# kongzhecn/OMG

Hardware: NVIDIA H100
Metric: 1024^2 images/sec @30 steps, 2 concepts (higher is better)
Workload: dtype f16

## Files before the change

### omg_b200/csrc/gemm_tc.cu

```cuda
#include <cuda_fp16.h>
#include <stdlib.h>
#include <string.h>

#include <algorithm>
#include <type_traits>

#include "../../include/omg_b200.h"
#include "elem.cuh"
#include "host_common.h"
#include "ptx.cuh"
#include "wgmma.cuh"

namespace omg {

constexpr int BM = 128;
constexpr int BK = 64;
constexpr int GEMM_THREADS = 384;

struct SegDev {
    int a_map, dx, dy, a_c0, k_blocks, b_k0, b_map;
};

struct alignas(64) GemmParams {
    CUtensorMap a_maps[OMG_MAX_A];
    CUtensorMap b_maps[2];
    SegDev segs[OMG_MAX_SEGS];
    int n_segs;
    int units;
    int n_units;
    int tw, th, tiles_w, tiles_h;
    int img_w, img_h, img_b;
    int N, N_out;
    void* out;
    long long out_sw, out_sh, out_sb;
    const void* bias;
    const void* rowvec;
    int rowvec_ld;
    const void* residual;
    int residual_ld;
    int act_silu;
    float* stats_out;
    int stats_unit_planes;
    const float* stats_in;
    int stats_parts;
    long long stats_rows;
    float ln_inv_dim, ln_eps;
    const float* col_c1;
    const float* col_c2;
    int n_col_groups;
    long long col_group_end[8];
    int w_group_rows;
    const float* residual_f32;
    long long residual_f32_ld;
    float* out_f32;
    long long out_f32_ld;
    float4* col_stats;
    int cs_rb0, cs_rb_total;
};

template <int UN, bool CS>
struct GemmCfg {
    static constexpr int ACC = UN;
    static constexpr int A_BYTES = BM * BK * 2;
    static constexpr int B_BYTES = UN * BK * 2;
    static constexpr int STAGE_BYTES = A_BYTES + B_BYTES;
    static constexpr int VEC_BYTES = 2 * 2 * UN * 4;
    static constexpr int CS_BYTES = CS ? 2 * 8 * (UN / 2) * 16 : 0;
    static constexpr int BARS_BYTES = 256;
    static constexpr int BUDGET = 227 * 1024 - 1024  - VEC_BYTES - CS_BYTES - BARS_BYTES;
    static constexpr int STAGES_RAW = BUDGET / STAGE_BYTES;
    static constexpr int STAGES = STAGES_RAW > 8 ? 8 : STAGES_RAW;
    static constexpr int SMEM_BYTES = 1024 + STAGES * STAGE_BYTES + VEC_BYTES + CS_BYTES + BARS_BYTES;
    static_assert(STAGES >= 2, "shared memory budget");
    static_assert((2 * STAGES + 2) * 8 <= BARS_BYTES, "barrier space");
};

__device__ __forceinline__ float gelu_exact(float x) { return 0.5f * x * (1.0f + erff(x * 0.70710678118654752f)); }

template <typename T, int WN>
__device__ __forceinline__ void wgmma_ss(float* d, uint64_t da, uint64_t db) {
    if constexpr (std::is_same_v<T, __nv_bfloat16>) {
        if constexpr (WN == 64) wgmma_ss_n64_bf16(*reinterpret_cast<float(*)[32]>(d), da, db, 1u);
        else if constexpr (WN == 128) wgmma_ss_n128_bf16(*reinterpret_cast<float(*)[64]>(d), da, db, 1u);
        else wgmma_ss_n160_bf16(*reinterpret_cast<float(*)[80]>(d), da, db, 1u);
    } else {
        if constexpr (WN == 64) wgmma_ss_n64(*reinterpret_cast<float(*)[32]>(d), da, db, 1u);
        else if constexpr (WN == 128) wgmma_ss_n128(*reinterpret_cast<float(*)[64]>(d), da, db, 1u);
        else wgmma_ss_n160(*reinterpret_cast<float(*)[80]>(d), da, db, 1u);
    }
}

template <int STAGES>
__device__ __forceinline__ void ring_advance(int& stage, uint32_t& phase, int n) {
    stage += n;
    const int wraps = stage / STAGES;
    stage -= wraps * STAGES;
    phase ^= (uint32_t)wraps & 1u;
}

template <typename T, int UN, int EPI, int FEAT>
__global__ void __launch_bounds__(GEMM_THREADS, 1) gemm_tc_kernel(const __grid_constant__ GemmParams p) {
    using T2 = pair_t<T>;
    constexpr bool kStats = FEAT >= 1, kExtra = FEAT >= 2;
    static_assert(EPI != OMG_EPI_GEGLU || UN == 160, "GEGLU runs on 160-wide units");
    using Cfg = GemmCfg<UN, kStats>;
    constexpr int STAGES = Cfg::STAGES;
    constexpr int NJ = UN / 8;
    extern __shared__ __align__(1024) uint8_t smem_raw[];
    uint8_t* smem = reinterpret_cast<uint8_t*>((reinterpret_cast<uintptr_t>(smem_raw) + 1023) & ~uintptr_t(1023));
    float* s_vec = reinterpret_cast<float*>(smem + STAGES * Cfg::STAGE_BYTES);
    float4* s_cs_all = reinterpret_cast<float4*>(s_vec + 2 * 2 * UN);
    uint64_t* full_bar = reinterpret_cast<uint64_t*>(reinterpret_cast<uint8_t*>(s_cs_all) + Cfg::CS_BYTES);
    uint64_t* empty_bar = full_bar + STAGES;
    uint64_t* turn_bar = empty_bar + STAGES;

    const int warp = threadIdx.x >> 5;
    const int lane = threadIdx.x & 31;
    const int tiles_per_img = p.tiles_w * p.tiles_h;

    if (warp == 8 && lane == 0) {
        for (int i = 0; i < OMG_MAX_A; ++i) tma_prefetch_desc(&p.a_maps[i]);
        tma_prefetch_desc(&p.b_maps[0]);
        tma_prefetch_desc(&p.b_maps[1]);
        for (int i = 0; i < STAGES; ++i) {
            mbar_init(&full_bar[i], 1);
            mbar_init(&empty_bar[i], 1);
        }
        mbar_init(&turn_bar[0], 1);
        mbar_init(&turn_bar[1], 1);
        fence_barrier_init();
    }
    __syncthreads();
    griddep_launch_dependents();
    griddep_wait();

    if (warp >= 8) {
        asm volatile("setmaxnreg.dec.sync.aligned.u32 40;");
        if (warp == 8 && lane == 0) {
            int stage = 0;
            uint32_t phase = 0;
            for (int u = blockIdx.x; u < p.units; u += gridDim.x) {
                const int m_tile = u / p.n_units, nu = u % p.n_units;
                const int b = m_tile / tiles_per_img;
                const int rem = m_tile % tiles_per_img;
                const int h0 = (rem / p.tiles_w) * p.th, w0 = (rem % p.tiles_w) * p.tw;
                int n0 = nu * UN;
                if (p.w_group_rows > 0) {
                    const long long tile_pix0 = ((long long)b * p.img_h + h0) * p.img_w + w0;
                    for (int g2 = 0; g2 + 1 < p.n_col_groups; ++g2)
                        if (tile_pix0 >= p.col_group_end[g2]) n0 += p.w_group_rows;
                }
                for (int s = 0; s < p.n_segs; ++s) {
                    const SegDev sg = p.segs[s];
                    for (int kb = 0; kb < sg.k_blocks; ++kb) {
                        mbar_wait_nocall(&empty_bar[stage], phase ^ 1);
                        uint8_t* a_dst = smem + stage * Cfg::STAGE_BYTES;
                        uint8_t* b_dst = a_dst + Cfg::A_BYTES;
                        mbar_arrive_expect_tx(&full_bar[stage], Cfg::STAGE_BYTES);
                        tma_load_4d(a_dst, &p.a_maps[sg.a_map], &full_bar[stage], sg.a_c0 + kb * BK, w0 + sg.dx, h0 + sg.dy, b);
                        tma_load_2d(b_dst, &p.b_maps[sg.b_map], &full_bar[stage], sg.b_k0 + kb * BK, n0);
                        if (++stage == STAGES) {
                            stage = 0;
                            phase ^= 1;
                        }
                    }
                }
            }
        }
        return;
    }

    asm volatile("setmaxnreg.inc.sync.aligned.u32 232;");
    const int wg = warp >> 2;
    const int wi = warp & 3;
    const int g = lane >> 2, c = lane & 3;
    const int wtid = threadIdx.x & 127;
    float* s_bias = s_vec + wg * (2 * UN);
    float* s_c1 = s_bias + UN;
    float4* s_cs = s_cs_all + wg * (8 * (UN / 2));
    int unit_kb = 0;
    for (int s = 0; s < p.n_segs; ++s) unit_kb += p.segs[s].k_blocks;
    int stage = 0;
    uint32_t phase = 0;
    if (wg == 1) ring_advance<STAGES>(stage, phase, unit_kb);
    uint32_t turn_phase = wg == 0 ? 1u : 0u;
    float acc[Cfg::ACC];

    for (int u = blockIdx.x + wg * gridDim.x; u < p.units; u += 2 * gridDim.x) {
        const int m_tile = u / p.n_units, nu = u % p.n_units;
        const int n0 = nu * UN;
        const int b = m_tile / tiles_per_img;
        const int rem = m_tile % tiles_per_img;
        const int h0 = (rem / p.tiles_w) * p.th, w0 = (rem % p.tiles_w) * p.tw;
        const bool ln = p.stats_in != nullptr;

        named_bar_sync(1 + wg, 128);
        {
            size_t cg = 0;
            if (ln && p.n_col_groups > 1) {
                const long long tile_pix0 = ((long long)b * p.img_h + h0) * p.img_w + w0;
                for (int g2 = 0; g2 + 1 < p.n_col_groups; ++g2)
                    if (tile_pix0 >= p.col_group_end[g2]) cg = g2 + 1;
                cg *= (size_t)p.N;
            }
            for (int j = wtid; j < UN; j += 128) {
                float v = 0.f, c1 = 0.f;
                const int n = n0 + j;
                if (n < p.N) {
                    if (ln) {
                        v = p.col_c2[cg + n];
                        c1 = p.col_c1[cg + n];
                    } else {
                        if (p.bias) v += to_f32(static_cast<const T*>(p.bias)[n]);
                        if (p.rowvec && b < p.img_b) v += to_f32(static_cast<const T*>(p.rowvec)[(size_t)b * p.rowvec_ld + n]);
                    }
                }
                s_bias[j] = v;
                s_c1[j] = c1;
            }
        }
        named_bar_sync(1 + wg, 128);

#pragma unroll
        for (int i = 0; i < Cfg::ACC; ++i) acc[i] = 0.f;
        mbar_wait_nocall(&turn_bar[wg], turn_phase);
        turn_phase ^= 1;
        int prev_stage = -1;
        for (int s = 0; s < p.n_segs; ++s) {
            const int kbs = p.segs[s].k_blocks;
            for (int kb = 0; kb < kbs; ++kb) {
                mbar_wait_nocall(&full_bar[stage], phase);
                const uint32_t a_addr = smem_u32(smem + stage * Cfg::STAGE_BYTES);
                const uint32_t b_addr = a_addr + Cfg::A_BYTES;
                wgmma_fence();
#pragma unroll
                for (int k = 0; k < BK / 16; ++k) {
                    const uint64_t b_desc = gmma_desc_sw128(b_addr + k * 32, 1024, 16);
#pragma unroll
                    for (int i = 0; i < 2; ++i)
                        wgmma_ss<T, UN>(acc + i * (UN / 2), gmma_desc_sw128(a_addr + i * (64 * BK * 2) + k * 32, 1024, 16), b_desc);
                }
                wgmma_commit();
                wgmma_wait<1>();
                if (prev_stage >= 0 && wtid == 0) mbar_arrive(&empty_bar[prev_stage]);
                prev_stage = stage;
                if (++stage == STAGES) {
                    stage = 0;
                    phase ^= 1;
                }
            }
        }
        if (wtid == 0) mbar_arrive(&turn_bar[wg ^ 1]);
        wgmma_wait<0>();
        reg_fence(acc);
        if (wtid == 0) mbar_arrive(&empty_bar[prev_stage]);
        ring_advance<STAGES>(stage, phase, unit_kb);

#pragma unroll
        for (int blk = 0; blk < 2; ++blk) {
            float* a = acc + blk * (UN / 2);
            float row_sum[2] = {0.f, 0.f}, row_sq[2] = {0.f, 0.f};
            bool valid[2];
            size_t pix[2];
            T* orow[2];
            float ln_a[2] = {1.f, 1.f}, ln_k[2] = {0.f, 0.f};
#pragma unroll
            for (int h = 0; h < 2; ++h) {
                const int et = blk * 64 + wi * 16 + g + 8 * h;
                const int ph = h0 + et / p.tw, pw = w0 + et % p.tw;
                valid[h] = (ph < p.img_h) && (pw < p.img_w) && (b < p.img_b);
                pix[h] = ((size_t)b * p.img_h + ph) * p.img_w + pw;
                orow[h] = static_cast<T*>(p.out) + (long long)b * p.out_sb + (long long)ph * p.out_sh + (long long)pw * p.out_sw;
                if (ln && valid[h]) {
                    float sa = 0.f, sq = 0.f;
                    for (int t = 0; t < p.stats_parts; ++t) {
                        const float2 st = __ldg(reinterpret_cast<const float2*>(p.stats_in) + (size_t)t * p.stats_rows + pix[h]);
                        sa += st.x;
                        sq += st.y;
                    }
                    const float mu = sa * p.ln_inv_dim;
                    ln_a[h] = rsqrtf(fmaxf(sq * p.ln_inv_dim - mu * mu, 0.f) + p.ln_eps);
                    ln_k[h] = -ln_a[h] * mu;
                }
            }
            float4* cs_slot = s_cs + (size_t)(blk * 4 + wi) * (UN / 2);
#pragma unroll
            for (int J = 0; J < NJ; ++J) {
                const int col = 8 * J + 2 * c;
                const int n = n0 + col;
                float x[2][2];
// ... 8 lines not shown
#pragma unroll
                    for (int h = 0; h < 2; ++h) {
                        const float o = x[h][0] * gelu_exact(x[h][1]);
                        const float o_nb = __shfl_down_sync(0xffffffffu, o, 1);
                        if ((c & 1) == 0 && valid[h] && n < p.N)
                            *reinterpret_cast<T2*>(orow[h] + (n >> 1)) = from_f32x2<T>(o, o_nb);
                    }
                } else {
                    if constexpr (kExtra) {
#pragma unroll
                        for (int h = 0; h < 2; ++h)
#pragma unroll
                            for (int e = 0; e < 2; ++e) {
                                float v = x[h][e];
                                if (p.act_silu == 1) {
                                    v = v / (1.0f + __expf(-v));
                                } else if (p.act_silu == 2) {
                                    v = v / (1.0f + __expf(-1.702f * v));
                                } else if (p.act_silu == 3) {
                                    v = gelu_exact(v);
                                } else if (p.act_silu == 4) {
                                    const float u = 0.7978845608028654f * fmaf(0.044715f * v * v, v, v);
                                    v = 0.5f * v * (2.0f - __fdividef(2.0f, 1.0f + __expf(2.0f * u)));
                                } else if (p.act_silu == 5) {
                                    v = fmaxf(v, 0.f);
                                }
                                x[h][e] = v;
                            }
                    }
                    float4 cs = make_float4(0.f, 0.f, 0.f, 0.f);
#pragma unroll
                    for (int h = 0; h < 2; ++h) {
                        const bool ok = valid[h] && n < p.N;
                        if (ok && p.residual != nullptr) {
                            const float2 r = to_f32x2(*reinterpret_cast<const T2*>(static_cast<const T*>(p.residual) + pix[h] * (size_t)p.residual_ld + n));
                            x[h][0] += r.x;
                            x[h][1] += r.y;
                        }
                        if constexpr (kExtra) {
                            if (ok && p.residual_f32 != nullptr) {
                                const float2 r = *reinterpret_cast<const float2*>(p.residual_f32 + pix[h] * (size_t)p.residual_f32_ld + n);
                                x[h][0] += r.x;
                                x[h][1] += r.y;
                            }
                            if (ok && p.out_f32 != nullptr)
                                *reinterpret_cast<float2*>(p.out_f32 + pix[h] * (size_t)p.out_f32_ld + n) = make_float2(x[h][0], x[h][1]);
                        }
                        if (ok) {
                            row_sum[h] += x[h][0] + x[h][1];
                            row_sq[h] = fmaf(x[h][0], x[h][0], fmaf(x[h][1], x[h][1], row_sq[h]));
                        }
                        const T2 o = from_f32x2<T>(x[h][0], x[h][1]);
                        if (ok) *reinterpret_cast<T2*>(orow[h] + n) = o;
                        if constexpr (kStats) {
                            const float2 f = valid[h] ? to_f32x2(o) : make_float2(0.f, 0.f);
                            cs.x += f.x;
                            cs.y = fmaf(f.x, f.x, cs.y);
                            cs.z += f.y;
                            cs.w = fmaf(f.y, f.y, cs.w);
                        }
                    }
                    if constexpr (kStats) {
                        if (p.col_stats != nullptr) {
#pragma unroll
                            for (int off = 4; off < 32; off <<= 1) {
                                cs.x += __shfl_xor_sync(0xffffffffu, cs.x, off);
                                cs.y += __shfl_xor_sync(0xffffffffu, cs.y, off);
                                cs.z += __shfl_xor_sync(0xffffffffu, cs.z, off);
                                cs.w += __shfl_xor_sync(0xffffffffu, cs.w, off);
                            }
                            if (g == 0) cs_slot[4 * J + c] = cs;
                        }
                    }
                }
            }
            if constexpr (EPI != OMG_EPI_GEGLU) {
                if (p.stats_out != nullptr) {
                    float2* so = reinterpret_cast<float2*>(p.stats_out);
                    const int kp = p.stats_unit_planes, plane0 = nu * kp;
#pragma unroll
                    for (int h = 0; h < 2; ++h) {
                        float s = row_sum[h], q = row_sq[h];
                        s += __shfl_xor_sync(0xffffffffu, s, 1);
                        q += __shfl_xor_sync(0xffffffffu, q, 1);
                        s += __shfl_xor_sync(0xffffffffu, s, 2);
                        q += __shfl_xor_sync(0xffffffffu, q, 2);
                        if (c == 0 && valid[h]) {
                            so[(size_t)plane0 * p.stats_rows + pix[h]] = make_float2(s, q);
                            for (int t = 1; t < kp; ++t) so[(size_t)(plane0 + t) * p.stats_rows + pix[h]] = make_float2(0.f, 0.f);
                        }
                    }
                }
            }
            if constexpr (EPI != OMG_EPI_GEGLU && kStats) {
                if (p.col_stats != nullptr) {
                    named_bar_sync(3 + wg * 2 + (wi >> 1), 64);
                    const int q = blk * 2 + (wi >> 1);
                    const float4* s0 = s_cs + (size_t)(blk * 4 + (wi & 2)) * (UN / 2);
                    const float4* s1 = s0 + UN / 2;
                    if (b < p.img_b) {
                        const size_t rb = (size_t)b * p.cs_rb_total + p.cs_rb0 + (size_t)rem * 4 + q;
                        for (int cp = (wi & 1) * 32 + lane; cp < UN / 2; cp += 64) {
                            const int col = n0 + 2 * cp;
                            if (col < p.N) {
                                const float4 u4 = s0[cp], w4 = s1[cp];
                                p.col_stats[(rb * p.N + col) >> 1] = make_float4(u4.x + w4.x, u4.y + w4.y, u4.z + w4.z, u4.w + w4.w);
                            }
                        }
                    }
                }
            }
        }
    }
}

static int view_to_tmap(CUtensorMap* m, const omg_view4& v, CUtensorMapDataType dt, uint32_t box_c, uint32_t box_w,
                        uint32_t box_h, CUtensorMapSwizzle sw) {
    const uint64_t dims[4] = {(uint64_t)v.C, (uint64_t)v.W, (uint64_t)v.H, (uint64_t)v.B};
    const uint64_t strides[4] = {1, (uint64_t)v.sw, (uint64_t)v.sh, (uint64_t)v.sb};
    const uint32_t box[4] = {box_c, box_w, box_h, 1};
    return make_tmap(m, dt, v.ptr, 4, dims, strides, box, sw);
}

template <typename T, int UN, int EPI, int FEAT>
static int launch_gemm_f(const GemmParams& p, cudaStream_t stream) {
    using Cfg = GemmCfg<UN, (FEAT >= 1)>;
    static bool configured = false;
    static int num_sms = 0;
    if (!configured) {
        OMG_CUDA(cudaFuncSetAttribute(gemm_tc_kernel<T, UN, EPI, FEAT>, cudaFuncAttributeMaxDynamicSharedMemorySize,
                                      Cfg::SMEM_BYTES));
        int dev = 0;
        OMG_CUDA(cudaGetDevice(&dev));
        OMG_CUDA(cudaDeviceGetAttribute(&num_sms, cudaDevAttrMultiProcessorCount, dev));
        configured = true;
    }
    const int grid = std::min(p.units, num_sms);
    OMG_CUDA(launch_pdl(gemm_tc_kernel<T, UN, EPI, FEAT>, dim3(grid), dim3(GEMM_THREADS), Cfg::SMEM_BYTES, stream, p));
    return check_launch("gemm_tc_kernel");
}

template <int UN, int EPI>
static int launch_gemm(const GemmParams& p, cudaStream_t stream) {
    if constexpr (EPI == OMG_EPI_GEGLU) {
        return launch_gemm_f<__half, UN, EPI, 0>(p, stream);
    } else {
        if (p.act_silu != 0 || p.residual_f32 != nullptr || p.out_f32 != nullptr) return launch_gemm_f<__half, UN, EPI, 2>(p, stream);
        if (p.col_stats != nullptr) return launch_gemm_f<__half, UN, EPI, 1>(p, stream);
        return launch_gemm_f<__half, UN, EPI, 0>(p, stream);
    }
}

constexpr int PLAN_SMS = 132;
constexpr double TILE_OVERHEAD = 48.0;
static double tile_time(long tiles, double cols) {
    return (double)((tiles + PLAN_SMS - 1) / PLAN_SMS) * (cols + TILE_OVERHEAD);
}

constexpr long K_PLAN_LONG = 1000;
static int pick_block_n(int N, int epilogue, long m_tiles, long k_plan) {
    if (epilogue == OMG_EPI_GEGLU) return 256;
    const int cands[5] = {256, 160, 128, 64, 160};
    int best = 256;
    double best_t = 1e30;
    for (int i = 0; i < 5; ++i) {
        const bool pair = i == 4;
        if (pair && (k_plan < 16 || m_tiles < 2)) continue;
        const long nt = (N + cands[i] - 1) / cands[i];
        const long mt = pair ? (m_tiles + 1) / 2 : m_tiles;
        const double t = tile_time(nt * mt, pair ? 2.0 * cands[i] : cands[i]);
        if (t < best_t - 1e-9) {
            best_t = t;
            best = cands[i];
        }
    }
    return best;
}

}

using namespace omg;

// ... 43 lines not shown
    const bool silu = d->epilogue == OMG_EPI_SILU;
    const int act = silu ? 1 : (d->epilogue == OMG_EPI_QUICK_GELU ? 2 : (d->epilogue == OMG_EPI_GELU ? 3 : (d->epilogue == OMG_EPI_GELU_TANH ? 4 :
                    (d->epilogue == OMG_EPI_RELU ? 5 : 0))));
    OMG_CHECK(d->epilogue == OMG_EPI_NONE || geglu || act, "omg_gemm: unknown epilogue %d", d->epilogue);
    const int N_out = geglu ? d->N / 2 : d->N;
    OMG_CHECK(d->d.C == N_out, "omg_gemm: output view has %d channels, expected %d", d->d.C, N_out);
    OMG_CHECK(!geglu || (d->N % 64 == 0 && !d->residual && !d->rowvec),
              "omg_gemm: GEGLU needs N %% 64 == 0 and no residual/rowvec");
    OMG_CHECK(!d->residual || (N_out % 32 == 0 && d->residual_ld % 8 == 0),
              "omg_gemm: residual needs N %% 32 == 0 and ld %% 8 == 0");

    GemmParams p;
    memset(&p, 0, sizeof(p));
    const int W = d->d.W, H = d->d.H, B = d->d.B;
    OMG_CHECK(W >= 1 && H >= 1 && B >= 1, "omg_gemm: empty output grid");
    int tw = 128;
    while (tw / 2 >= W && tw > 1) tw /= 2;
    const int th = 128 / tw;
    p.tw = tw;
    p.th = th;
    p.tiles_w = (W + tw - 1) / tw;
    p.tiles_h = (H + th - 1) / th;
    p.img_w = W;
    p.img_h = H;
    p.img_b = B;
    const int m_tiles = p.tiles_w * p.tiles_h * B;
    p.N = d->N;
    p.N_out = N_out;
    const long k_blocks_hint = (long)(d->Ktot + (d->w2 ? d->K2tot : 0)) / 64;
    int bn = d->block_n ? d->block_n
                        : pick_block_n(d->N, d->epilogue, m_tiles, d->row_stats_out ? K_PLAN_LONG : k_blocks_hint);
    OMG_CHECK(bn == 64 || bn == 128 || bn == 160 || bn == 256 || bn == 320, "omg_gemm: block_n=%d unsupported", bn);
    OMG_CHECK(bn != 320 || (!geglu && d->N % 320 == 0), "omg_gemm: block_n=320 needs N %% 320 == 0 and no GEGLU");
    OMG_CHECK(d->cta_pair == 0 || d->cta_pair == 1 || d->cta_pair == 3, "omg_gemm: cta_pair=%d unsupported (0, 1 or 3)",
              d->cta_pair);
    if (geglu) bn = 256;
    const int unit_n = geglu ? 160 : (bn > 160 ? bn / 2 : bn);
    const int tile_units = geglu ? 1 : bn / unit_n;
    p.n_units = geglu ? (d->N + 159) / 160 : (d->N + bn - 1) / bn * tile_units;
    p.units = m_tiles * p.n_units;
    p.stats_unit_planes = (bn == 320 ? 4 : 2) / tile_units;
    p.bias = d->bias;
    p.rowvec = d->rowvec;
    p.rowvec_ld = d->rowvec_ld;
    p.residual = d->residual;
    p.residual_ld = d->residual_ld;
    p.act_silu = act;
    p.stats_out = static_cast<float*>(d->row_stats_out);
    p.stats_in = static_cast<const float*>(d->row_stats_in);
    p.stats_parts = d->row_stats_parts;
    p.stats_rows = d->row_stats_stride > 0 ? d->row_stats_stride : (long long)W * H * B;
    p.ln_inv_dim = d->ln_dim > 0 ? 1.0f / (float)d->ln_dim : 0.f;
    p.ln_eps = d->ln_eps;
    p.col_c1 = static_cast<const float*>(d->col_c1);
    p.col_c2 = static_cast<const float*>(d->col_c2);
    p.n_col_groups = d->n_col_groups > 0 ? d->n_col_groups : 1;
    p.w_group_rows = d->w_group_planes > 0 ? d->N : 0;
    OMG_CHECK(d->w_group_planes == 0 || d->w_group_planes == p.n_col_groups, "omg_gemm: w_group_planes must equal n_col_groups");
    OMG_CHECK(p.n_col_groups <= 8, "omg_gemm: at most 8 column-vector row groups");
    OMG_CHECK(d->w_group_planes == 0 || !d->w2, "omg_gemm: weight planes do not extend to the second weight matrix (w2)");
    const long long img_pix = (long long)W * H;
    for (int i = 0; i < 8; ++i) {
        p.col_group_end[i] = d->col_group_end[i];
        if (i + 1 >= p.n_col_groups) continue;
        if (H > 1)
            OMG_CHECK(d->col_group_end[i] % img_pix == 0,
                      "omg_gemm: row-group boundary %lld is inside an image of the %d x %d output grid (boundaries are "
                      "multiples of %lld pixels)", (long long)d->col_group_end[i], W, H, img_pix);
        else
            OMG_CHECK(d->col_group_end[i] % 128 == 0, "omg_gemm: row-group boundary %lld is not a multiple of the 128-row tile",
                      (long long)d->col_group_end[i]);
    }
    OMG_CHECK(!p.stats_in || (p.col_c1 && p.col_c2 && d->ln_dim > 0 && d->row_stats_parts >= 1 && !d->rowvec),
              "omg_gemm: folded LayerNorm needs col_c1, col_c2, ln_dim, row_stats_parts and no rowvec");
    OMG_CHECK(!p.stats_out || !geglu, "omg_gemm: row statistics cannot be emitted by the GEGLU epilogue");
    p.residual_f32 = static_cast<const float*>(d->residual_f32);
    p.residual_f32_ld = d->residual_f32_ld;
    p.out_f32 = static_cast<float*>(d->out_f32);
    p.out_f32_ld = d->out_f32_ld;
    OMG_CHECK((!p.residual_f32 && !p.out_f32) || (!geglu && d->N % 32 == 0 && !(d->residual && d->residual_f32)),
              "omg_gemm: fp32 residual / output twins need a non-GEGLU epilogue, N %% 32 == 0, and replace the fp16 residual");
    OMG_CHECK((!p.residual_f32 || d->residual_f32_ld % 4 == 0) && (!p.out_f32 || d->out_f32_ld % 4 == 0),
              "omg_gemm: fp32 twin row strides must be multiples of 4");
    OMG_CHECK((!p.residual_f32 && !p.out_f32) || (d->d.sw == d->d.C && d->d.sh == (int64_t)d->d.sw * W && d->d.sb == d->d.sh * H),
              "omg_gemm: fp32 twins need a contiguous output view (rows are indexed by pixel)");
    p.col_stats = static_cast<float4*>(d->col_stats_out);
    p.cs_rb0 = d->col_stats_rb0;
    p.cs_rb_total = d->col_stats_rb_total;
    OMG_CHECK(!p.col_stats || (!geglu && d->N % 32 == 0 && d->col_stats_rb0 >= 0 &&
                               d->col_stats_rb0 + p.tiles_w * p.tiles_h * 4 <= d->col_stats_rb_total),
              "omg_gemm: column statistics need a non-GEGLU epilogue, N %% 32 == 0 and rb0 + blocks <= rb_total");
    OMG_CHECK((!p.stats_out && !p.stats_in) || (d->d.sw == d->d.C && d->d.sh == (int64_t)d->d.sw * W && d->d.sb == d->d.sh * H),
              "omg_gemm: row statistics need a contiguous output view");

    for (int i = 0; i < d->n_a; ++i) {
        OMG_CHECK(d->a[i].ptr != nullptr, "omg_gemm: A view %d is null", i);
        if (view_to_tmap(&p.a_maps[i], d->a[i], tdt, BK, tw, th, CU_TENSOR_MAP_SWIZZLE_128B)) return 1;
    }
    for (int i = d->n_a; i < OMG_MAX_A; ++i) p.a_maps[i] = p.a_maps[0];
    {
        const uint64_t planes = d->w_group_planes > 0 ? (uint64_t)d->w_group_planes : 1;
        const uint64_t dims[2] = {(uint64_t)d->Ktot, (uint64_t)d->N * planes};
        const uint64_t strides[2] = {1, (uint64_t)d->Ktot};
        const uint32_t box[2] = {BK, (uint32_t)unit_n};
        if (make_tmap(&p.b_maps[0], tdt, d->w, 2, dims, strides, box, CU_TENSOR_MAP_SWIZZLE_128B)) return 1;
        p.b_maps[1] = p.b_maps[0];
    }
    if (d->w2 != nullptr) {
        OMG_CHECK(d->K2tot >= 8 && d->K2tot % 8 == 0, "omg_gemm: K2tot=%d must be a positive multiple of 8", d->K2tot);
        const uint64_t dims[2] = {(uint64_t)d->K2tot, (uint64_t)d->N};
        const uint64_t strides[2] = {1, (uint64_t)d->K2tot};
        const uint32_t box[2] = {BK, (uint32_t)unit_n};
        if (make_tmap(&p.b_maps[1], tdt, d->w2, 2, dims, strides, box, CU_TENSOR_MAP_SWIZZLE_128B)) return 1;
    }
    OMG_CHECK(d->d.sw % 2 == 0 && d->d.sh % 2 == 0 && d->d.sb % 2 == 0 && (reinterpret_cast<uintptr_t>(d->d.ptr) & 3) == 0,
              "omg_gemm: output view must be 4 B aligned per pixel");
    p.out = const_cast<void*>(d->d.ptr);
    p.out_sw = d->d.sw;
    p.out_sh = d->d.sh;
    p.out_sb = d->d.sb;

    p.n_segs = d->n_segs;
    for (int s = 0; s < d->n_segs; ++s) {
        const omg_seg& sg = d->segs[s];
        OMG_CHECK(sg.a_idx >= 0 && sg.a_idx < d->n_a, "omg_gemm: segment %d references A view %d", s, sg.a_idx);
        OMG_CHECK(sg.k_len > 0 && sg.a_c0 >= 0 && sg.b_k0 >= 0 && sg.a_c0 + sg.k_len <= d->a[sg.a_idx].C,
                  "omg_gemm: segment %d has a bad K range", s);
        OMG_CHECK(sg.b_idx == 0 || (sg.b_idx == 1 && d->w2 != nullptr), "omg_gemm: segment %d has a bad b_idx", s);
        const int ktot_s = sg.b_idx ? d->K2tot : d->Ktot;
        OMG_CHECK(sg.b_k0 + sg.k_len <= ktot_s, "omg_gemm: segment %d exceeds weight K (%d + %d > %d)", s, sg.b_k0,
                  sg.k_len, ktot_s);
        OMG_CHECK(sg.k_len % BK == 0 || sg.a_c0 + sg.k_len == d->a[sg.a_idx].C,
                  "omg_gemm: segment %d: K tail must end at the A view's last channel", s);
        p.segs[s] = SegDev{sg.a_idx, sg.dx, sg.dy, sg.a_c0, (sg.k_len + BK - 1) / BK, sg.b_k0, sg.b_idx};
    }

    if (bf16) {
        switch (unit_n) {
            case 64: return launch_gemm_f<__nv_bfloat16, 64, OMG_EPI_NONE, 0>(p, stream);
            case 128: return launch_gemm_f<__nv_bfloat16, 128, OMG_EPI_NONE, 0>(p, stream);
            default: return launch_gemm_f<__nv_bfloat16, 160, OMG_EPI_NONE, 0>(p, stream);
        }
    }
    if (geglu) return launch_gemm<160, OMG_EPI_GEGLU>(p, stream);
    switch (unit_n) {
        case 64: return launch_gemm<64, OMG_EPI_NONE>(p, stream);
        case 128: return launch_gemm<128, OMG_EPI_NONE>(p, stream);
        default: return launch_gemm<160, OMG_EPI_NONE>(p, stream);
    }
}

extern "C" int omg_gemm(const omg_gemm_desc* d, void* stream_) {
    const int rc = gemm_impl(d, stream_);
    if (rc == 0 && ::omg::plan_recording()) {
        const omg_gemm_desc c = *d;
        ::omg::plan_note([c](void* s) { return gemm_impl(&c, s); });
    }
    return rc;
}
```

### omg_b200/csrc/ptx.cuh

```cuda
#pragma once
#include <cuda.h>
#include <cuda_fp16.h>
#include <cuda_runtime.h>
#include <stdint.h>
#include <stdio.h>

namespace omg {

__device__ __forceinline__ uint32_t smem_u32(const void* p) {
    return static_cast<uint32_t>(__cvta_generic_to_shared(p));
}

__device__ __forceinline__ uint32_t lane_id() { return threadIdx.x & 31; }

__device__ __forceinline__ bool elect_one() {
    uint32_t pred;
    asm volatile(
        "{\n\t.reg .pred p;\n\t"
        "elect.sync _|p, 0xffffffff;\n\t"
        "selp.u32 %0, 1, 0, p;\n\t}\n"
        : "=r"(pred));
    return pred != 0;
}

__device__ __forceinline__ void griddep_launch_dependents() { asm volatile("griddepcontrol.launch_dependents;" ::: "memory"); }
__device__ __forceinline__ void griddep_wait() { asm volatile("griddepcontrol.wait;" ::: "memory"); }

__device__ __forceinline__ void mbar_init(uint64_t* bar, uint32_t count) {
    asm volatile("mbarrier.init.shared::cta.b64 [%0], %1;" ::"r"(smem_u32(bar)), "r"(count));
}
__device__ __forceinline__ void fence_barrier_init() {
    asm volatile("fence.mbarrier_init.release.cluster;" ::: "memory");
}
__device__ __forceinline__ void fence_proxy_async_smem() {
    asm volatile("fence.proxy.async.shared::cta;" ::: "memory");
}
__device__ __forceinline__ void mbar_arrive_expect_tx(uint64_t* bar, uint32_t bytes) {
    asm volatile("mbarrier.arrive.expect_tx.shared::cta.b64 _, [%0], %1;" ::"r"(smem_u32(bar)), "r"(bytes)
                 : "memory");
}
__device__ __forceinline__ void mbar_arrive(uint64_t* bar) {
    asm volatile("mbarrier.arrive.shared::cta.b64 _, [%0];" ::"r"(smem_u32(bar)) : "memory");
}
__device__ __forceinline__ bool mbar_try_wait(uint64_t* bar, uint32_t parity) {
    uint32_t ok;
    asm volatile(
        "{\n\t.reg .pred p;\n\t"
        "mbarrier.try_wait.parity.shared::cta.b64 p, [%1], %2;\n\t"
        "selp.u32 %0, 1, 0, p;\n\t}\n"
        : "=r"(ok)
        : "r"(smem_u32(bar)), "r"(parity)
        : "memory");
    return ok != 0;
}
#ifndef OMG_MBAR_TIMEOUT_CYCLES
#define OMG_MBAR_TIMEOUT_CYCLES (4000000000LL)
#endif
#ifndef OMG_MBAR_SUSPEND_NS
#define OMG_MBAR_SUSPEND_NS 20000
#endif
__device__ __forceinline__ bool mbar_try_wait_long(uint64_t* bar, uint32_t parity) {
    uint32_t ok;
    asm volatile(
        "{\n\t.reg .pred p;\n\t"
        "mbarrier.try_wait.parity.shared::cta.b64 p, [%1], %2, %3;\n\t"
        "selp.u32 %0, 1, 0, p;\n\t}\n"
        : "=r"(ok)
        : "r"(smem_u32(bar)), "r"(parity), "r"((uint32_t)OMG_MBAR_SUSPEND_NS)
        : "memory");
    return ok != 0;
}
__device__ __forceinline__ void mbar_wait(uint64_t* bar, uint32_t parity) {
    if (mbar_try_wait(bar, parity)) return;
    const long long t0 = clock64();
    uint32_t spins = 0;
    while (!mbar_try_wait_long(bar, parity)) {
        if ((++spins & 0x3FF) == 0 && clock64() - t0 > OMG_MBAR_TIMEOUT_CYCLES) {
            printf("omg: mbarrier timeout block=(%d,%d,%d) thread=%d bar=%u parity=%u\n", (int)blockIdx.x,
                   (int)blockIdx.y, (int)blockIdx.z, (int)threadIdx.x, smem_u32(bar), parity);
            __trap();
        }
    }
}

__device__ __forceinline__ void mbar_wait_nocall(uint64_t* bar, uint32_t parity) {
    if (mbar_try_wait(bar, parity)) return;
    const long long t0 = clock64();
    uint32_t spins = 0;
    while (!mbar_try_wait_long(bar, parity))
        if ((++spins & 0x3FF) == 0 && clock64() - t0 > OMG_MBAR_TIMEOUT_CYCLES) __trap();
}

__device__ __forceinline__ float fast_exp2(float x) {
    float y;
    asm("ex2.approx.ftz.f32 %0, %1;" : "=f"(y) : "f"(x));
    return y;
}

__device__ __forceinline__ void tma_prefetch_desc(const CUtensorMap* m) {
    asm volatile("prefetch.tensormap [%0];" ::"l"(reinterpret_cast<uint64_t>(m)) : "memory");
}
__device__ __forceinline__ void tma_load_2d(void* smem_dst, const CUtensorMap* m, uint64_t* bar, int c0, int c1) {
    asm volatile(
        "cp.async.bulk.tensor.2d.shared::cluster.global.mbarrier::complete_tx::bytes [%0], [%1, {%3, %4}], [%2];"
        ::"r"(smem_u32(smem_dst)), "l"(reinterpret_cast<uint64_t>(m)), "r"(smem_u32(bar)), "r"(c0), "r"(c1)
        : "memory");
}
__device__ __forceinline__ void tma_load_3d(void* smem_dst, const CUtensorMap* m, uint64_t* bar, int c0, int c1,
                                            int c2) {
    asm volatile(
        "cp.async.bulk.tensor.3d.shared::cluster.global.mbarrier::complete_tx::bytes [%0], [%1, {%3, %4, %5}], [%2];"
        ::"r"(smem_u32(smem_dst)), "l"(reinterpret_cast<uint64_t>(m)), "r"(smem_u32(bar)), "r"(c0), "r"(c1), "r"(c2)
        : "memory");
}
__device__ __forceinline__ void tma_load_4d(void* smem_dst, const CUtensorMap* m, uint64_t* bar, int c0, int c1,
                                            int c2, int c3) {
    asm volatile(
        "cp.async.bulk.tensor.4d.shared::cluster.global.mbarrier::complete_tx::bytes [%0], [%1, {%3, %4, %5, %6}], "
        "[%2];"
        ::"r"(smem_u32(smem_dst)), "l"(reinterpret_cast<uint64_t>(m)), "r"(smem_u32(bar)), "r"(c0), "r"(c1), "r"(c2),
        "r"(c3)
        : "memory");
}
__device__ __forceinline__ void tma_store_3d(const CUtensorMap* m, const void* smem_src, int c0, int c1, int c2) {
    asm volatile("cp.async.bulk.tensor.3d.global.shared::cta.bulk_group [%0, {%2, %3, %4}], [%1];" ::"l"(
                     reinterpret_cast<uint64_t>(m)),
                 "r"(smem_u32(smem_src)), "r"(c0), "r"(c1), "r"(c2)
                 : "memory");
}
__device__ __forceinline__ void tma_store_4d(const CUtensorMap* m, const void* smem_src, int c0, int c1, int c2,
                                             int c3) {
    asm volatile("cp.async.bulk.tensor.4d.global.shared::cta.bulk_group [%0, {%2, %3, %4, %5}], [%1];" ::"l"(
                     reinterpret_cast<uint64_t>(m)),
                 "r"(smem_u32(smem_src)), "r"(c0), "r"(c1), "r"(c2), "r"(c3)
                 : "memory");
}
__device__ __forceinline__ void tma_store_commit() { asm volatile("cp.async.bulk.commit_group;" ::: "memory"); }
template <int N>
__device__ __forceinline__ void tma_store_wait_read() {
    asm volatile("cp.async.bulk.wait_group.read %0;" ::"n"(N) : "memory");
// ... 8 lines not shown
    d |= static_cast<uint64_t>((smem_addr & 0x3FFFF) >> 4);
    d |= static_cast<uint64_t>((lbo_bytes >> 4) & 0x3FFF) << 16;
    d |= static_cast<uint64_t>((sbo_bytes >> 4) & 0x3FFF) << 32;
    d |= static_cast<uint64_t>(1) << 62;
    return d;
}
__device__ __forceinline__ uint64_t gmma_desc_sw32(uint32_t smem_addr) {
    uint64_t d = 0;
    d |= static_cast<uint64_t>((smem_addr & 0x3FFFF) >> 4);
    d |= static_cast<uint64_t>(256 >> 4) << 16;
    d |= static_cast<uint64_t>(256 >> 4) << 32;
    d |= static_cast<uint64_t>(3) << 62;
    return d;
}
__device__ __forceinline__ void wgmma_fence() { asm volatile("wgmma.fence.sync.aligned;" ::: "memory"); }
__device__ __forceinline__ void wgmma_commit() { asm volatile("wgmma.commit_group.sync.aligned;" ::: "memory"); }
template <int N>
__device__ __forceinline__ void wgmma_wait() {
    asm volatile("wgmma.wait_group.sync.aligned %0;" ::"n"(N) : "memory");
}
template <int N>
__device__ __forceinline__ void reg_fence(float (&r)[N]) {
#pragma unroll
    for (int i = 0; i < N; ++i) asm volatile("" : "+f"(r[i])::"memory");
}
__device__ __forceinline__ void named_bar_sync(int id, int count) {
    asm volatile("bar.sync %0, %1;" ::"r"(id), "r"(count) : "memory");
}

__device__ __forceinline__ void st_shared_v4(uint32_t addr, uint32_t a, uint32_t b, uint32_t c, uint32_t d) {
    asm volatile("st.shared.v4.b32 [%0], {%1, %2, %3, %4};" ::"r"(addr), "r"(a), "r"(b), "r"(c), "r"(d) : "memory");
}

__device__ __forceinline__ uint32_t pack_half2(float a, float b) {
    __half2 h = __floats2half2_rn(a, b);
    return *reinterpret_cast<uint32_t*>(&h);
}

}
```

Before: 0.1969.

## Pair CTAs in 2-CTA clusters and multicast the weight tiles via TMA

Adds an optional 2-CTA cluster mode for the persistent wgmma GEMM. Two CTAs take adjacent M tiles with the same N unit, and each loads half of the shared B (weight) tile, multicasting it to both CTAs. Empty barriers now need an arrival from both CTAs, and the producer drains the ring before exiting. The mode is on by default when N > 1280 and the row-group boundaries are even. It halves weight traffic from L2 per CTA, at the cost of cross-CTA coupling, cluster scheduling limits and extra remote barrier arrivals.

New measurement: 0.1997, median of 6. +1.4%, better.

```diff
diff --git a/omg_b200/csrc/gemm_tc.cu b/omg_b200/csrc/gemm_tc.cu
--- a/omg_b200/csrc/gemm_tc.cu
+++ b/omg_b200/csrc/gemm_tc.cu
@@ -26,6 +26,7 @@
     CUtensorMap b_maps[2];
     SegDev segs[OMG_MAX_SEGS];
     int n_segs;
+    int pair;
     int units;
     int n_units;
     int tw, th, tiles_w, tiles_h;
@@ -117,6 +118,9 @@
     const int warp = threadIdx.x >> 5;
     const int lane = threadIdx.x & 31;
     const int tiles_per_img = p.tiles_w * p.tiles_h;
+    const int pair = p.pair;
+    const uint32_t rank = pair == 2 ? cluster_ctarank() : 0u;
+    const int cluster = blockIdx.x / pair, clusters = gridDim.x / pair;
 
     if (warp == 8 && lane == 0) {
         for (int i = 0; i < OMG_MAX_A; ++i) tma_prefetch_desc(&p.a_maps[i]);
@@ -124,29 +128,38 @@
         tma_prefetch_desc(&p.b_maps[1]);
         for (int i = 0; i < STAGES; ++i) {
             mbar_init(&full_bar[i], 1);
-            mbar_init(&empty_bar[i], 1);
+            mbar_init(&empty_bar[i], pair);
         }
         mbar_init(&turn_bar[0], 1);
         mbar_init(&turn_bar[1], 1);
         fence_barrier_init();
     }
-    __syncthreads();
+    if (pair == 2) {
+        cluster_arrive();
+        cluster_wait();
+    } else {
+        __syncthreads();
+    }
     griddep_launch_dependents();
     griddep_wait();
 
     if (warp >= 8) {
         asm volatile("setmaxnreg.dec.sync.aligned.u32 40;");
         if (warp == 8 && lane == 0) {
+            constexpr int HALF_ROWS = UN / 2, HALF_BYTES = HALF_ROWS * BK * 2;
             int stage = 0;
             uint32_t phase = 0;
-            for (int u = blockIdx.x; u < p.units; u += gridDim.x) {
-                const int m_tile = u / p.n_units, nu = u % p.n_units;
+            for (int u = cluster; u < p.units; u += clusters) {
+                const int m_pair = u / p.n_units, nu = u % p.n_units;
+                const int m_tile = m_pair * pair + (int)rank;
                 const int b = m_tile / tiles_per_img;
                 const int rem = m_tile % tiles_per_img;
                 const int h0 = (rem / p.tiles_w) * p.th, w0 = (rem % p.tiles_w) * p.tw;
                 int n0 = nu * UN;
                 if (p.w_group_rows > 0) {
-                    const long long tile_pix0 = ((long long)b * p.img_h + h0) * p.img_w + w0;
+                    const int m0 = m_pair * pair, rem0 = m0 % tiles_per_img;
+                    const long long tile_pix0 = ((long long)(m0 / tiles_per_img) * p.img_h + (rem0 / p.tiles_w) * p.th) * p.img_w +
+                                                (rem0 % p.tiles_w) * p.tw;
                     for (int g2 = 0; g2 + 1 < p.n_col_groups; ++g2)
                         if (tile_pix0 >= p.col_group_end[g2]) n0 += p.w_group_rows;
                 }
@@ -156,14 +169,27 @@
                         mbar_wait_nocall(&empty_bar[stage], phase ^ 1);
                         uint8_t* a_dst = smem + stage * Cfg::STAGE_BYTES;
                         uint8_t* b_dst = a_dst + Cfg::A_BYTES;
+                        const int k0 = sg.b_k0 + kb * BK;
                         mbar_arrive_expect_tx(&full_bar[stage], Cfg::STAGE_BYTES);
                         tma_load_4d(a_dst, &p.a_maps[sg.a_map], &full_bar[stage], sg.a_c0 + kb * BK, w0 + sg.dx, h0 + sg.dy, b);
-                        tma_load_2d(b_dst, &p.b_maps[sg.b_map], &full_bar[stage], sg.b_k0 + kb * BK, n0);
+                        if (pair == 2) {
+                            tma_load_2d_multicast(b_dst + rank * HALF_BYTES, &p.b_maps[sg.b_map], &full_bar[stage], k0,
+                                                  n0 + (int)rank * HALF_ROWS, 0x3);
+                        } else {
+                            tma_load_2d(b_dst, &p.b_maps[sg.b_map], &full_bar[stage], k0, n0);
+                        }
                         if (++stage == STAGES) {
                             stage = 0;
                             phase ^= 1;
                         }
                     }
+                }
+            }
+            for (int i = 0; i < STAGES; ++i) {
+                mbar_wait_nocall(&empty_bar[stage], phase ^ 1);
+                if (++stage == STAGES) {
+                    stage = 0;
+                    phase ^= 1;
                 }
             }
         }
@@ -185,9 +211,13 @@
     if (wg == 1) ring_advance<STAGES>(stage, phase, unit_kb);
     uint32_t turn_phase = wg == 0 ? 1u : 0u;
     float acc[Cfg::ACC];
-
-    for (int u = blockIdx.x + wg * gridDim.x; u < p.units; u += 2 * gridDim.x) {
-        const int m_tile = u / p.n_units, nu = u % p.n_units;
+    auto release = [&](int s) {
+        mbar_arrive(&empty_bar[s]);
+        if (pair == 2) mbar_arrive_cluster(&empty_bar[s], rank ^ 1u);
+    };
+
+    for (int u = cluster + wg * clusters; u < p.units; u += 2 * clusters) {
+        const int m_tile = (u / p.n_units) * pair + (int)rank, nu = u % p.n_units;
         const int n0 = nu * UN;
         const int b = m_tile / tiles_per_img;
         const int rem = m_tile % tiles_per_img;
@@ -242,7 +272,7 @@
                 }
                 wgmma_commit();
                 wgmma_wait<1>();
-                if (prev_stage >= 0 && wtid == 0) mbar_arrive(&empty_bar[prev_stage]);
+                if (prev_stage >= 0 && wtid == 0) release(prev_stage);
                 prev_stage = stage;
                 if (++stage == STAGES) {
                     stage = 0;
@@ -253,7 +283,7 @@
         if (wtid == 0) mbar_arrive(&turn_bar[wg ^ 1]);
         wgmma_wait<0>();
         reg_fence(acc);
-        if (wtid == 0) mbar_arrive(&empty_bar[prev_stage]);
+        if (wtid == 0) release(prev_stage);
         ring_advance<STAGES>(stage, phase, unit_kb);
 
 #pragma unroll
@@ -424,17 +454,31 @@
 static int launch_gemm_f(const GemmParams& p, cudaStream_t stream) {
     using Cfg = GemmCfg<UN, (FEAT >= 1)>;
     static bool configured = false;
-    static int num_sms = 0;
+    static int num_sms = 0, num_pairs = 0;
     if (!configured) {
         OMG_CUDA(cudaFuncSetAttribute(gemm_tc_kernel<T, UN, EPI, FEAT>, cudaFuncAttributeMaxDynamicSharedMemorySize,
                                       Cfg::SMEM_BYTES));
         int dev = 0;
         OMG_CUDA(cudaGetDevice(&dev));
         OMG_CUDA(cudaDeviceGetAttribute(&num_sms, cudaDevAttrMultiProcessorCount, dev));
+        cudaLaunchConfig_t cfg = {};
+        cudaLaunchAttribute attr;
+        attr.id = cudaLaunchAttributeClusterDimension;
+        attr.val.clusterDim.x = 2;
+        attr.val.clusterDim.y = 1;
+        attr.val.clusterDim.z = 1;
+        cfg.gridDim = dim3(2 * num_sms);
+        cfg.blockDim = dim3(GEMM_THREADS);
+        cfg.dynamicSmemBytes = Cfg::SMEM_BYTES;
+        cfg.attrs = &attr;
+        cfg.numAttrs = 1;
+        OMG_CUDA(cudaOccupancyMaxActiveClusters(&num_pairs, gemm_tc_kernel<T, UN, EPI, FEAT>, &cfg));
         configured = true;
     }
-    const int grid = std::min(p.units, num_sms);
-    OMG_CUDA(launch_pdl(gemm_tc_kernel<T, UN, EPI, FEAT>, dim3(grid), dim3(GEMM_THREADS), Cfg::SMEM_BYTES, stream, p));
+    OMG_CHECK(p.pair == 1 || num_pairs >= 1, "gemm_tc_kernel: no 2-CTA cluster fits on this device");
+    const int grid = p.pair * std::min(p.units, p.pair == 2 ? num_pairs : num_sms);
+    OMG_CUDA(launch_cluster(gemm_tc_kernel<T, UN, EPI, FEAT>, dim3(grid), dim3(GEMM_THREADS), Cfg::SMEM_BYTES, stream, p.pair,
+                            p));
     return check_launch("gemm_tc_kernel");
 }
 
@@ -555,13 +599,11 @@
                         : pick_block_n(d->N, d->epilogue, m_tiles, d->row_stats_out ? K_PLAN_LONG : k_blocks_hint);
     OMG_CHECK(bn == 64 || bn == 128 || bn == 160 || bn == 256 || bn == 320, "omg_gemm: block_n=%d unsupported", bn);
     OMG_CHECK(bn != 320 || (!geglu && d->N % 320 == 0), "omg_gemm: block_n=320 needs N %% 320 == 0 and no GEGLU");
-    OMG_CHECK(d->cta_pair == 0 || d->cta_pair == 1 || d->cta_pair == 3, "omg_gemm: cta_pair=%d unsupported (0, 1 or 3)",
-              d->cta_pair);
+    OMG_CHECK(d->cta_pair >= 0 && d->cta_pair <= 3, "omg_gemm: cta_pair=%d unsupported (0, 1, 2 or 3)", d->cta_pair);
     if (geglu) bn = 256;
     const int unit_n = geglu ? 160 : (bn > 160 ? bn / 2 : bn);
     const int tile_units = geglu ? 1 : bn / unit_n;
     p.n_units = geglu ? (d->N + 159) / 160 : (d->N + bn - 1) / bn * tile_units;
-    p.units = m_tiles * p.n_units;
     p.stats_unit_planes = (bn == 320 ? 4 : 2) / tile_units;
     p.bias = d->bias;
     p.rowvec = d->rowvec;
@@ -594,6 +636,12 @@
             OMG_CHECK(d->col_group_end[i] % 128 == 0, "omg_gemm: row-group boundary %lld is not a multiple of the 128-row tile",
                       (long long)d->col_group_end[i]);
     }
+    p.pair = d->cta_pair == 2 || (d->cta_pair == 0 && d->N > 1280) ? 2 : 1;
+    for (int i = 0; i + 1 < p.n_col_groups && d->w_group_planes > 0; ++i) {
+        const long long e = d->col_group_end[i];
+        if (((e / img_pix) * p.tiles_w * p.tiles_h + (e % img_pix) / tw) % 2 != 0) p.pair = 1;
+    }
+    p.units = (m_tiles + p.pair - 1) / p.pair * p.n_units;
     OMG_CHECK(!p.stats_in || (p.col_c1 && p.col_c2 && d->ln_dim > 0 && d->row_stats_parts >= 1 && !d->rowvec),
               "omg_gemm: folded LayerNorm needs col_c1, col_c2, ln_dim, row_stats_parts and no rowvec");
     OMG_CHECK(!p.stats_out || !geglu, "omg_gemm: row statistics cannot be emitted by the GEGLU epilogue");
@@ -625,7 +673,7 @@
         const uint64_t planes = d->w_group_planes > 0 ? (uint64_t)d->w_group_planes : 1;
         const uint64_t dims[2] = {(uint64_t)d->Ktot, (uint64_t)d->N * planes};
         const uint64_t strides[2] = {1, (uint64_t)d->Ktot};
-        const uint32_t box[2] = {BK, (uint32_t)unit_n};
+        const uint32_t box[2] = {BK, (uint32_t)(unit_n / p.pair)};
         if (make_tmap(&p.b_maps[0], tdt, d->w, 2, dims, strides, box, CU_TENSOR_MAP_SWIZZLE_128B)) return 1;
         p.b_maps[1] = p.b_maps[0];
     }
@@ -633,7 +681,7 @@
         OMG_CHECK(d->K2tot >= 8 && d->K2tot % 8 == 0, "omg_gemm: K2tot=%d must be a positive multiple of 8", d->K2tot);
         const uint64_t dims[2] = {(uint64_t)d->K2tot, (uint64_t)d->N};
         const uint64_t strides[2] = {1, (uint64_t)d->K2tot};
-        const uint32_t box[2] = {BK, (uint32_t)unit_n};
+        const uint32_t box[2] = {BK, (uint32_t)(unit_n / p.pair)};
         if (make_tmap(&p.b_maps[1], tdt, d->w2, 2, dims, strides, box, CU_TENSOR_MAP_SWIZZLE_128B)) return 1;
     }
     OMG_CHECK(d->d.sw % 2 == 0 && d->d.sh % 2 == 0 && d->d.sb % 2 == 0 && (reinterpret_cast<uintptr_t>(d->d.ptr) & 3) == 0,
diff --git a/omg_b200/csrc/ptx.cuh b/omg_b200/csrc/ptx.cuh
--- a/omg_b200/csrc/ptx.cuh
+++ b/omg_b200/csrc/ptx.cuh
@@ -26,6 +26,14 @@
 __device__ __forceinline__ void griddep_launch_dependents() { asm volatile("griddepcontrol.launch_dependents;" ::: "memory"); }
 __device__ __forceinline__ void griddep_wait() { asm volatile("griddepcontrol.wait;" ::: "memory"); }
 
+__device__ __forceinline__ uint32_t cluster_ctarank() {
+    uint32_t r;
+    asm volatile("mov.u32 %0, %%cluster_ctarank;" : "=r"(r));
+    return r;
+}
+__device__ __forceinline__ void cluster_arrive() { asm volatile("barrier.cluster.arrive.release.aligned;" ::: "memory"); }
+__device__ __forceinline__ void cluster_wait() { asm volatile("barrier.cluster.wait.acquire.aligned;" ::: "memory"); }
+
 __device__ __forceinline__ void mbar_init(uint64_t* bar, uint32_t count) {
     asm volatile("mbarrier.init.shared::cta.b64 [%0], %1;" ::"r"(smem_u32(bar)), "r"(count));
 }
@@ -41,6 +49,14 @@
 }
 __device__ __forceinline__ void mbar_arrive(uint64_t* bar) {
     asm volatile("mbarrier.arrive.shared::cta.b64 _, [%0];" ::"r"(smem_u32(bar)) : "memory");
+}
+__device__ __forceinline__ void mbar_arrive_cluster(uint64_t* bar, uint32_t cta_rank) {
+    asm volatile(
+        "{\n\t.reg .b32 remote;\n\t"
+        "mapa.shared::cluster.u32 remote, %0, %1;\n\t"
+        "mbarrier.arrive.shared::cluster.b64 _, [remote];\n\t}\n"
+        ::"r"(smem_u32(bar)), "r"(cta_rank)
+        : "memory");
 }
 __device__ __forceinline__ bool mbar_try_wait(uint64_t* bar, uint32_t parity) {
     uint32_t ok;
@@ -106,6 +122,14 @@
         ::"r"(smem_u32(smem_dst)), "l"(reinterpret_cast<uint64_t>(m)), "r"(smem_u32(bar)), "r"(c0), "r"(c1)
         : "memory");
 }
+__device__ __forceinline__ void tma_load_2d_multicast(void* smem_dst, const CUtensorMap* m, uint64_t* bar, int c0, int c1,
+                                                      uint16_t cta_mask) {
+    asm volatile(
+        "cp.async.bulk.tensor.2d.shared::cluster.global.mbarrier::complete_tx::bytes.multicast::cluster"
+        " [%0], [%1, {%3, %4}], [%2], %5;"
+        ::"r"(smem_u32(smem_dst)), "l"(reinterpret_cast<uint64_t>(m)), "r"(smem_u32(bar)), "r"(c0), "r"(c1), "h"(cta_mask)
+        : "memory");
+}
 __device__ __forceinline__ void tma_load_3d(void* smem_dst, const CUtensorMap* m, uint64_t* bar, int c0, int c1,
                                             int c2) {
     asm volatile(
```

## Stage GEMM residual tile into shared memory via TMA from a dedicated producer warp

Applied to the files above, without the earlier changes.

Adds a TMA tensor map for the residual and a second producer warp that loads each unit's residual tile into a swizzled shared buffer, double-buffered with its own full/empty mbarriers. The epilogue reads the residual from shared memory instead of scattered global loads, so the residual fetch overlaps the mainloop. The cost is shared memory taken from the stage budget, which can reduce pipeline depth, plus extra barrier traffic. A single residual buffer is shared across the two consumer warpgroups and ordered by the turn barriers.

Result: faster. 0.1955 before, 0.2014 after (median of 6 runs) (+3.1%).

```diff
diff --git a/omg_b200/csrc/gemm_tc.cu b/omg_b200/csrc/gemm_tc.cu
--- a/omg_b200/csrc/gemm_tc.cu
+++ b/omg_b200/csrc/gemm_tc.cu
@@ -56,9 +56,11 @@
     long long out_f32_ld;
     float4* col_stats;
     int cs_rb0, cs_rb_total;
+    CUtensorMap res_map;
 };
 
-template <int UN, bool CS>
+constexpr int RES_BOX_BYTES = BM * 32 * 2;
+template <int UN, bool CS, bool RES = false>
 struct GemmCfg {
     static constexpr int ACC = UN;
     static constexpr int A_BYTES = BM * BK * 2;
@@ -66,13 +68,15 @@
     static constexpr int STAGE_BYTES = A_BYTES + B_BYTES;
     static constexpr int VEC_BYTES = 2 * 2 * UN * 4;
     static constexpr int CS_BYTES = CS ? 2 * 8 * (UN / 2) * 16 : 0;
+    static constexpr int RES_BYTES = RES ? (UN / 32) * RES_BOX_BYTES : 0;
     static constexpr int BARS_BYTES = 256;
-    static constexpr int BUDGET = 227 * 1024 - 1024  - VEC_BYTES - CS_BYTES - BARS_BYTES;
+    static constexpr int BUDGET = 227 * 1024 - 1024  - RES_BYTES - VEC_BYTES - CS_BYTES - BARS_BYTES;
     static constexpr int STAGES_RAW = BUDGET / STAGE_BYTES;
     static constexpr int STAGES = STAGES_RAW > 8 ? 8 : STAGES_RAW;
-    static constexpr int SMEM_BYTES = 1024 + STAGES * STAGE_BYTES + VEC_BYTES + CS_BYTES + BARS_BYTES;
+    static constexpr int SMEM_BYTES = 1024 + STAGES * STAGE_BYTES + RES_BYTES + VEC_BYTES + CS_BYTES + BARS_BYTES;
     static_assert(STAGES >= 2, "shared memory budget");
-    static_assert((2 * STAGES + 2) * 8 <= BARS_BYTES, "barrier space");
+    static_assert(STAGE_BYTES % 1024 == 0, "the residual buffer follows the stages on a 1024 B boundary");
+    static_assert((2 * STAGES + 5) * 8 <= BARS_BYTES, "barrier space");
 };
 
 __device__ __forceinline__ float gelu_exact(float x) { return 0.5f * x * (1.0f + erff(x * 0.70710678118654752f)); }
@@ -98,21 +102,25 @@
     phase ^= (uint32_t)wraps & 1u;
 }
 
-template <typename T, int UN, int EPI, int FEAT>
+template <typename T, int UN, int EPI, int FEAT, bool RES = false>
 __global__ void __launch_bounds__(GEMM_THREADS, 1) gemm_tc_kernel(const __grid_constant__ GemmParams p) {
     using T2 = pair_t<T>;
     constexpr bool kStats = FEAT >= 1, kExtra = FEAT >= 2;
     static_assert(EPI != OMG_EPI_GEGLU || UN == 160, "GEGLU runs on 160-wide units");
-    using Cfg = GemmCfg<UN, kStats>;
+    static_assert(!RES || (std::is_same_v<T, __half> && EPI == OMG_EPI_NONE && FEAT <= 1), "staged residual: fp16, FEAT 0 / 1");
+    using Cfg = GemmCfg<UN, kStats, RES>;
     constexpr int STAGES = Cfg::STAGES;
     constexpr int NJ = UN / 8;
     extern __shared__ __align__(1024) uint8_t smem_raw[];
     uint8_t* smem = reinterpret_cast<uint8_t*>((reinterpret_cast<uintptr_t>(smem_raw) + 1023) & ~uintptr_t(1023));
-    float* s_vec = reinterpret_cast<float*>(smem + STAGES * Cfg::STAGE_BYTES);
+    uint8_t* s_res = smem + STAGES * Cfg::STAGE_BYTES;
+    float* s_vec = reinterpret_cast<float*>(s_res + Cfg::RES_BYTES);
     float4* s_cs_all = reinterpret_cast<float4*>(s_vec + 2 * 2 * UN);
     uint64_t* full_bar = reinterpret_cast<uint64_t*>(reinterpret_cast<uint8_t*>(s_cs_all) + Cfg::CS_BYTES);
     uint64_t* empty_bar = full_bar + STAGES;
     uint64_t* turn_bar = empty_bar + STAGES;
+    uint64_t* res_full = turn_bar + 2;
+    uint64_t* res_empty = res_full + 2;
 
     const int warp = threadIdx.x >> 5;
     const int lane = threadIdx.x & 31;
@@ -128,6 +136,12 @@
         }
         mbar_init(&turn_bar[0], 1);
         mbar_init(&turn_bar[1], 1);
+        if constexpr (RES) {
+            tma_prefetch_desc(&p.res_map);
+            mbar_init(&res_full[0], 1);
+            mbar_init(&res_full[1], 1);
+            mbar_init(res_empty, 4);
+        }
         fence_barrier_init();
     }
     __syncthreads();
@@ -167,6 +181,22 @@
                 }
             }
         }
+        if constexpr (RES) {
+            if (warp == 9 && lane == 0) {
+                int j = 0;
+                for (int u = blockIdx.x; u < p.units; u += gridDim.x, ++j) {
+                    const int m_tile = u / p.n_units, nu = u % p.n_units;
+                    const int b = m_tile / tiles_per_img;
+                    const int rem = m_tile % tiles_per_img;
+                    const int h0 = (rem / p.tiles_w) * p.th, w0 = (rem % p.tiles_w) * p.tw;
+                    mbar_wait_nocall(res_empty, (j & 1) ^ 1);
+                    mbar_arrive_expect_tx(&res_full[j & 1], Cfg::RES_BYTES);
+#pragma unroll
+                    for (int i = 0; i < UN / 32; ++i)
+                        tma_load_4d(s_res + i * RES_BOX_BYTES, &p.res_map, &res_full[j & 1], nu * UN + 32 * i, w0, h0, b);
+                }
+            }
+        }
         return;
     }
 
@@ -256,6 +286,8 @@
         if (wtid == 0) mbar_arrive(&empty_bar[prev_stage]);
         ring_advance<STAGES>(stage, phase, unit_kb);
 
+        const uint32_t res_row = (smem_u32(s_res) + (wi * 16 + g) * 64 + 4 * c) | ((g >> 1) << 4);
+        if constexpr (RES) mbar_wait_nocall(&res_full[wg], turn_phase ^ wg);
 #pragma unroll
         for (int blk = 0; blk < 2; ++blk) {
             float* a = acc + blk * (UN / 2);
@@ -330,7 +362,15 @@
 #pragma unroll
                     for (int h = 0; h < 2; ++h) {
                         const bool ok = valid[h] && n < p.N;
-                        if (ok && p.residual != nullptr) {
+                        if constexpr (RES) {
+                            const uint32_t rb = ld_shared_b32((res_row ^ ((J & 3) << 4)) + (J >> 2) * RES_BOX_BYTES + blk * 64 * 64 + h * 8 * 64);
+                            const T2 rv = *reinterpret_cast<const T2*>(&rb);
+                            if (ok) {
+                                const float2 r = to_f32x2(rv);
+                                x[h][0] += r.x;
+                                x[h][1] += r.y;
+                            }
+                        } else if (ok && p.residual != nullptr) {
                             const float2 r = to_f32x2(*reinterpret_cast<const T2*>(static_cast<const T*>(p.residual) + pix[h] * (size_t)p.residual_ld + n));
                             x[h][0] += r.x;
                             x[h][1] += r.y;
@@ -372,6 +412,12 @@
                     }
                 }
             }
+            if constexpr (RES) {
+                if (blk == 1) {
+                    __syncwarp();
+                    if (elect_one()) mbar_arrive(res_empty);
+                }
+            }
             if constexpr (EPI != OMG_EPI_GEGLU) {
                 if (p.stats_out != nullptr) {
                     float2* so = reinterpret_cast<float2*>(p.stats_out);
@@ -420,13 +466,13 @@
     return make_tmap(m, dt, v.ptr, 4, dims, strides, box, sw);
 }
 
-template <typename T, int UN, int EPI, int FEAT>
+template <typename T, int UN, int EPI, int FEAT, bool RES = false>
 static int launch_gemm_f(const GemmParams& p, cudaStream_t stream) {
-    using Cfg = GemmCfg<UN, (FEAT >= 1)>;
+    using Cfg = GemmCfg<UN, (FEAT >= 1), RES>;
     static bool configured = false;
     static int num_sms = 0;
     if (!configured) {
-        OMG_CUDA(cudaFuncSetAttribute(gemm_tc_kernel<T, UN, EPI, FEAT>, cudaFuncAttributeMaxDynamicSharedMemorySize,
+        OMG_CUDA(cudaFuncSetAttribute(gemm_tc_kernel<T, UN, EPI, FEAT, RES>, cudaFuncAttributeMaxDynamicSharedMemorySize,
                                       Cfg::SMEM_BYTES));
         int dev = 0;
         OMG_CUDA(cudaGetDevice(&dev));
@@ -434,18 +480,19 @@
         configured = true;
     }
     const int grid = std::min(p.units, num_sms);
-    OMG_CUDA(launch_pdl(gemm_tc_kernel<T, UN, EPI, FEAT>, dim3(grid), dim3(GEMM_THREADS), Cfg::SMEM_BYTES, stream, p));
+    OMG_CUDA(launch_pdl(gemm_tc_kernel<T, UN, EPI, FEAT, RES>, dim3(grid), dim3(GEMM_THREADS), Cfg::SMEM_BYTES, stream, p));
     return check_launch("gemm_tc_kernel");
 }
 
 template <int UN, int EPI>
-static int launch_gemm(const GemmParams& p, cudaStream_t stream) {
+static int launch_gemm(const GemmParams& p, bool res_staged, cudaStream_t stream) {
     if constexpr (EPI == OMG_EPI_GEGLU) {
         return launch_gemm_f<__half, UN, EPI, 0>(p, stream);
     } else {
         if (p.act_silu != 0 || p.residual_f32 != nullptr || p.out_f32 != nullptr) return launch_gemm_f<__half, UN, EPI, 2>(p, stream);
-        if (p.col_stats != nullptr) return launch_gemm_f<__half, UN, EPI, 1>(p, stream);
-        return launch_gemm_f<__half, UN, EPI, 0>(p, stream);
+        if (p.col_stats != nullptr)
+            return res_staged ? launch_gemm_f<__half, UN, EPI, 1, true>(p, stream) : launch_gemm_f<__half, UN, EPI, 1>(p, stream);
+        return res_staged ? launch_gemm_f<__half, UN, EPI, 0, true>(p, stream) : launch_gemm_f<__half, UN, EPI, 0>(p, stream);
     }
 }
 
@@ -665,11 +712,19 @@
             default: return launch_gemm_f<__nv_bfloat16, 160, OMG_EPI_NONE, 0>(p, stream);
         }
     }
-    if (geglu) return launch_gemm<160, OMG_EPI_GEGLU>(p, stream);
+    if (geglu) return launch_gemm<160, OMG_EPI_GEGLU>(p, false, stream);
+    bool res_staged = false;
+    if (d->residual != nullptr && (reinterpret_cast<uintptr_t>(d->residual) & 15) == 0) {
+        const uint64_t ld = (uint64_t)d->residual_ld;
+        const uint64_t dims[4] = {(uint64_t)N_out, (uint64_t)W, (uint64_t)H, (uint64_t)B};
+        const uint64_t strides[4] = {1, ld, ld * W, ld * W * H};
+        const uint32_t box[4] = {32, (uint32_t)tw, (uint32_t)th, 1};
+        res_staged = make_tmap(&p.res_map, tdt, d->residual, 4, dims, strides, box, CU_TENSOR_MAP_SWIZZLE_64B) == 0;
+    }
     switch (unit_n) {
-        case 64: return launch_gemm<64, OMG_EPI_NONE>(p, stream);
-        case 128: return launch_gemm<128, OMG_EPI_NONE>(p, stream);
-        default: return launch_gemm<160, OMG_EPI_NONE>(p, stream);
+        case 64: return launch_gemm<64, OMG_EPI_NONE>(p, res_staged, stream);
+        case 128: return launch_gemm<128, OMG_EPI_NONE>(p, res_staged, stream);
+        default: return launch_gemm<160, OMG_EPI_NONE>(p, res_staged, stream);
     }
 }
 
diff --git a/omg_b200/csrc/ptx.cuh b/omg_b200/csrc/ptx.cuh
--- a/omg_b200/csrc/ptx.cuh
+++ b/omg_b200/csrc/ptx.cuh
@@ -180,6 +180,12 @@
     asm volatile("st.shared.v4.b32 [%0], {%1, %2, %3, %4};" ::"r"(addr), "r"(a), "r"(b), "r"(c), "r"(d) : "memory");
 }
 
+__device__ __forceinline__ uint32_t ld_shared_b32(uint32_t addr) {
+    uint32_t v;
+    asm volatile("ld.shared.b32 %0, [%1];" : "=r"(v) : "r"(addr) : "memory");
+    return v;
+}
+
 __device__ __forceinline__ uint32_t pack_half2(float a, float b) {
     __half2 h = __floats2half2_rn(a, b);
     return *reinterpret_cast<uint32_t*>(&h);
```
